# sevagh/Zen

Measured on AMD Instinct MI355X. Metric: hops/sec (1024-hop HPR, 44.1 kHz mono), higher is better.
Workload: dtype f32

## Files before the change

zen_amd/__init__.py:

```python
from .lib import (
    FREQUENCY, OUTPUT_HARMONIC, OUTPUT_PERCUSSIVE, OUTPUT_RESIDUAL, TIME_ANTICAUSAL, TIME_CAUSAL,
    BoxFilterGPU, DeviceBuffer, Event, FFTC2CWrapperGPU, HPR, HPRIOffline, HPRRealtime, IOGPU, MedianFilterGPU, PinnedHost,
    ZenHipError, ZgException, blockrun_set, blockrun_stats, debug_poke, device_name, init, load, memcheck, run_plan, set_option, synchronize,
)
from .addon_build import beat as beat_build, cqt as cqt_build, live as live_build, multi as multi_build, pcm as pcm_build, pitch as pitch_build, ragged as ragged_build, repet as repet_build, repsim as repsim_build
```

zen_amd/addon_build.py:

```python
import glob
import os
import subprocess
import sys
from concurrent.futures import ThreadPoolExecutor

HERE = os.path.dirname(os.path.abspath(__file__))
ROOT = os.path.dirname(HERE)
BASE = os.path.join(HERE, "libzen_hip.so")
HIPCC = os.environ.get("HIPCC", "/opt/rocm/bin/hipcc")
FLAGS = ["--offload-arch=gfx950", "-O3", "-std=c++17", "-fPIC", "-ffp-contract=off", "-fno-fast-math", "-Wall",
         "-I", os.path.join(ROOT, "include")]


class Addon:

    def __init__(self, name, sources, extra_deps=(), build_demo=None, title=None, file_flags=None):
        self.name, self.SOURCES, self.build_demo, self.title = name, list(sources), build_demo, title or name
        self.SRC = os.path.join(HERE, name)
        self.OUT = os.path.join(HERE, "libzen_hip_%s.so" % name)
        self.OBJDIR = os.path.join(HERE, "build_" + name)
        self.FLAGS = FLAGS
        self.FILE_FLAGS = dict(file_flags or {})
        self.extra_deps = [os.path.join(HERE, *d.split("/")) for d in extra_deps]

    def deps(self):
        hdrs = [os.path.join(self.SRC, f) for f in os.listdir(self.SRC) if f.endswith(".h")]
        hdrs += glob.glob(os.path.join(HERE, "addon", "*.h")) + self.extra_deps
        hdrs.append(os.path.join(ROOT, "include", "zen_hip.h"))
        hdrs.append(os.path.abspath(__file__))
        return hdrs

    def objects(self):
        return [os.path.join(self.OBJDIR, s.replace(".hip", ".o")) for s in self.SOURCES]

    def _compile(self, src):
        obj = os.path.join(self.OBJDIR, src.replace(".hip", ".o"))
        srcp = os.path.join(self.SRC, src)
        newest = max(os.path.getmtime(p) for p in [srcp] + self.deps())
        if os.path.exists(obj) and os.path.getmtime(obj) >= newest:
            return obj, False
        subprocess.check_call([HIPCC] + self.FLAGS + self.FILE_FLAGS.get(src, []) + ["-c", srcp, "-o", obj])
        return obj, True

    def build(self, force=False, verbose=False):
        if not os.path.exists(BASE):
            raise RuntimeError("%s not built: zen_amd/build.py first (the %s library links against it)" % (BASE, self.title))
        os.makedirs(self.OBJDIR, exist_ok=True)
        if force:
            for f in os.listdir(self.OBJDIR):
                os.remove(os.path.join(self.OBJDIR, f))
        with ThreadPoolExecutor(max_workers=len(self.SOURCES)) as ex:
            res = list(ex.map(self._compile, self.SOURCES))
        if any(r[1] for r in res) or not os.path.exists(self.OUT) or os.path.getmtime(self.OUT) < os.path.getmtime(BASE):
            subprocess.check_call([HIPCC, "--offload-arch=gfx950", "-shared", "-fPIC", "-o", self.OUT] + [r[0] for r in res]
                                  + ["-L", HERE, "-lzen_hip", "-Wl,-rpath,$ORIGIN"])
            if verbose:
                print("built", self.OUT)
        if self.build_demo:
            self.build_demo(verbose)
        return self.OUT


def _build_demo(name, source, exe, verbose):
    src, out = os.path.join(HERE, name), os.path.join(HERE, "libzen_hip_%s.so" % name)
    srcs = [os.path.join(src, source), os.path.join(src, "zen_hip_%s.h" % name), os.path.join(HERE, "cli", "wav.h"), out]
    if os.path.exists(exe) and os.path.getmtime(exe) >= max(os.path.getmtime(p) for p in srcs):
        return exe
    os.makedirs(os.path.dirname(exe), exist_ok=True)
    subprocess.check_call([os.environ.get("CXX", "g++"), "-std=c++17", "-O2", "-Wall", "-ffp-contract=off", "-I", os.path.join(ROOT, "include"),
                           "-I", src, "-I", os.path.join(HERE, "cli"), srcs[0], "-o", exe, "-L", HERE, "-lzen_hip_" + name, "-lzen_hip",
                           "-Wl,-rpath,$ORIGIN/.."])
    if verbose:
        print("built", exe)
    return exe


DEMO = os.path.join(HERE, "bin", "pitch-track")
BEAT_DEMO = os.path.join(HERE, "bin", "beat-track")
STEMS_DEMO = os.path.join(HERE, "bin", "zen-stems")
REPET_DEMO = os.path.join(HERE, "bin", "zen-repet")
CQT_DEMO = os.path.join(HERE, "bin", "zen-cqt")
REPSIM_DEMO = os.path.join(HERE, "bin", "zen-repsim")


def build_demo(verbose=False):
    return _build_demo("pitch", "pitch_track.cpp", DEMO, verbose)


def build_beat_demo(verbose=False):
    return _build_demo("beat", "beat_track.cpp", BEAT_DEMO, verbose)


def build_stems_demo(verbose=False):
    return _build_demo("multi", "multi_stems.cpp", STEMS_DEMO, verbose)


def build_repet_demo(verbose=False):
    return _build_demo("repet", "repet_main.cpp", REPET_DEMO, verbose)


def build_cqt_demo(verbose=False):
    return _build_demo("cqt", "cqt_main.cpp", CQT_DEMO, verbose)


def build_repsim_demo(verbose=False):
    return _build_demo("repsim", "repsim_main.cpp", REPSIM_DEMO, verbose)


pcm = Addon("pcm", ["pcm_kernels.hip", "pcm_pipe.hip"], extra_deps=["csrc/host_pipe.h"], title="PCM")
ragged = Addon("ragged", ["ragged_kernels.hip", "ragged.hip"])
live = Addon("live", ["live_kernels.hip", "live.hip"])
pitch = Addon("pitch", ["pitch_kernels.hip", "pitch.hip"], build_demo=build_demo)
ADDONS = {a.name: a for a in (pcm, ragged, live, pitch)}
blockrun = Addon("blockrun", ["blockrun_kernel.hip", "blockrun.hip"],
                 extra_deps=["csrc/hpr_engine.h", "csrc/rt_fused.h", "csrc/common.h", "csrc/bounds.h", "csrc/memguard.h", "csrc/masks.h",
                             "csrc/fft_dev.h", "csrc/median47_core.h", "csrc/median_net.h"],
                 file_flags={"blockrun_kernel.hip": ["-mllvm", "-amdgpu-sched-strategy=max-ilp", "-mllvm", "-amdgpu-use-amdgpu-trackers=1",
                                                     "-DZEN_FFT_LDS_BARRIER", "-DZEN_FFT_FOLD_ADDR", "-Wno-unused-function"]})
ENGINE_ADDONS = {blockrun.name: blockrun}
beat = Addon("beat", ["beat_kernels.hip", "beat.hip"], build_demo=build_beat_demo)
multi = Addon("multi", ["multi_kernels.hip", "multi.hip"], extra_deps=["pcm/pcm_convert.h"], build_demo=build_stems_demo)
repet = Addon("repet", ["repet_kernels.hip", "repet.hip"], build_demo=build_repet_demo)
cqt = Addon("cqt", ["cqt_kernels.hip", "cqt.hip"], build_demo=build_cqt_demo)
repsim = Addon("repsim", ["repsim_kernels.hip", "repsim.hip"], build_demo=build_repsim_demo)
LATER_ADDONS = {beat.name: beat, multi.name: multi, repet.name: repet, cqt.name: cqt, repsim.name: repsim}
ALL_ADDONS = {**ADDONS, **ENGINE_ADDONS, **LATER_ADDONS}


if __name__ == "__main__":
    names = [a for a in sys.argv[1:] if not a.startswith("--")] or list(ALL_ADDONS)
    for n in names:
        ALL_ADDONS[n].build(force="--force" in sys.argv, verbose=True)
```

zen_amd/blockrun/blockrun.hip:

```cpp
#include "../csrc/hpr_engine.h"
#include "../csrc/masks.h"
#include "blockrun_kernel.h"
#include "zen_hip_blockrun.h"

#include <atomic>
#include <cstring>

using namespace zen_hip_impl;

namespace {

std::atomic<int> g_run_len{0}, g_min_items{4096}, g_off{0};
std::atomic<unsigned long long> g_routed{0}, g_forwarded{0};

struct ProfScope {
	zen_hip_hpr* e;
	int k;
	hipEvent_t e0 = nullptr, e1 = nullptr;
	ProfScope(zen_hip_hpr* e_, int k_)
	    : e(e_)
	    , k(k_)
	{
		if (!e->prof)
			return;
		if (!e->prof_pool.empty()) {
			e0 = e->prof_pool.back().first;
			e1 = e->prof_pool.back().second;
			e->prof_pool.pop_back();
		}
		else if (hipEventCreate(&e0) != hipSuccess || hipEventCreate(&e1) != hipSuccess) {
			e0 = e1 = nullptr;
			return;
		}
		(void)hipEventRecord(e0, e->stream);
	}
	~ProfScope()
	{
		if (!e0)
			return;
		(void)hipEventRecord(e1, e->stream);
		e->prof_pending.push_back({k, e0, e1});
		e->prof_launches[k] += 1;
	}
};

int device_slots(int* slots)
{
	static std::atomic<int> cached[64];
	int dev = 0;
	ZH_HIP(hipGetDevice(&dev));
	int v = (dev >= 0 && dev < 64) ? cached[dev].load() : 0;
	if (v == 0) {
		int cus = 0;
		ZH_HIP(hipDeviceGetAttribute(&cus, hipDeviceAttributeMultiprocessorCount, dev));
		v = 3 * (cus > 0 ? cus : 1);
		if (dev >= 0 && dev < 64)
			cached[dev].store(v);
	}
	*slots = v;
	return ZEN_HIP_OK;
}

bool takes(const zen_hip_hpr* h, const float* in, size_t n_hops, size_t in_stride, const float* harm, const float* perc,
           const float* resid, size_t out_stride)
{
	if (g_off.load() || !h || !in || !perc || harm || resid || n_hops == 0)
		return false;
	if (h->causality != ZEN_HIP_TIME_CAUSAL || h->log2n != 12 || h->mf != zen_blockrun::TAPS || h->hop != (size_t)zen_blockrun::HOP
	    || h->nfft != (size_t)zen_blockrun::NFFT || h->nwin != 2 * h->hop)
		return false;
	if (!h->out_p || h->out_h || h->out_r || h->soft || h->use_sse)
		return false;
	if ((h->drain[0] | h->drain[1] | h->drain[2]) || h->rows_stale || h->run_mode || h->res_idle_ms != 0 || h->res_active || h->dbg_stamps)
		return false;
	if (!h->d_Y[0] || !h->d_blk_need || !h->d_carry[0] || !h->d_mag || n_hops > h->max_hops)
		return false;
	if (h->n_streams * n_hops < (size_t)g_min_items.load() || h->n_streams * n_hops > 0x3fffffffu)
		return false;
	int inc = 0;
	if (hard_mask_threshold(h->beta, &inc) == 0.0)
		return false;
	const size_t S = h->n_streams;
	const char *in0 = (const char*)in, *in1 = (const char*)(in + (S - 1) * in_stride + n_hops * h->hop);
	const char *o0 = (const char*)perc, *o1 = (const char*)(perc + (S - 1) * out_stride + n_hops * h->hop);
	return !(o0 < in1 && in0 < o1);
}

}

extern "C" int zen_hip_blockrun_process(zen_hip_hpr_t h, const float* in_dev, size_t n_hops, size_t in_stride, float* harm, float* perc,
                                        float* resid, size_t out_stride)
{
	if (!takes(h, in_dev, n_hops, in_stride, harm, perc, resid, out_stride)) {
		g_forwarded.fetch_add(1);
		return zen_hip_hpr_process(h, in_dev, n_hops, in_stride, harm, perc, resid, out_stride);
	}
	g_routed.fetch_add(1);
	int slots = 0;
	ZH_TRY(device_slots(&slots));
	zen_blockrun::RunArgs a;
	memset(&a, 0, sizeof(a));
	a.in = in_dev;
	a.in_stride = (long long)in_stride;
	a.tail_prev = h->d_tail[h->tail_sel];
	a.tail_next = h->d_tail[h->tail_sel ^ 1];
	a.window = h->d_window;
	a.tw = h->d_tw;
	a.mag = h->d_mag;
	a.keep_mag_rows = (int)h->W - 1;
	a.ring_rows = h->ring_rows;
	a.row0 = h->abs_frame;
	a.n_frames = (int)n_hops;
	a.n_streams = (int)h->n_streams;
	a.prev_frames = (int)h->last_frames;
	a.carry = h->d_carry[0];
	a.Y = h->d_Y[0];
	a.y_stream_stride = (long long)(h->max_hops * h->nwin);
	a.out = perc;
	a.out_stride = (long long)out_stride;
	a.need = h->d_blk_need;
	a.cola = h->cola;
	int inc = 0;
	a.thr = hard_mask_threshold(h->beta, &inc);
	a.part = zen_blockrun_partition(a.n_streams, a.n_frames, slots, g_run_len.load());
	for (int o = 0; o < 3; ++o) {
		h->ready_valid[o] = false;
		h->direct_done[o] = false;
	}
	{
		ProfScope ps(h, zen_hip_hpr::K_FUSED);
		ZH_TRY(zen_blockrun::launch_run(a, h->stream));
	}
	{
		ProfScope ps(h, zen_hip_hpr::K_FINALIZE);
		ZH_TRY(zen_blockrun::launch_fixup(a, h->stream));
	}
	h->tail_sel ^= 1;
	h->abs_frame += (long long)n_hops;
	h->last_frames = n_hops;
	return ZEN_HIP_OK;
}

extern "C" int zen_hip_blockrun_set(const char* key, int value)
{
	if (!key || value < 0)
		ZH_FAIL(ZEN_HIP_E_BAD_ARG, "blockrun_set: null key or negative value");
	if (!strcmp(key, "run_len"))
		g_run_len.store(value);
	else if (!strcmp(key, "min_items"))
		g_min_items.store(value);
	else if (!strcmp(key, "off"))
		g_off.store(value);
	else
		ZH_FAIL(ZEN_HIP_E_BAD_ARG, "blockrun_set: unknown key '%s' (run_len, min_items, off)", key);
	return ZEN_HIP_OK;
}

extern "C" int zen_hip_blockrun_stats(unsigned long long* routed, unsigned long long* forwarded)
{
	if (routed)
		*routed = g_routed.load();
	if (forwarded)
		*forwarded = g_forwarded.load();
	return ZEN_HIP_OK;
}
```

zen_amd/blockrun/blockrun_kernel.h:

```cpp
#pragma once
#include <hip/hip_runtime.h>

#include "blockrun_partition.h"

namespace zen_blockrun {

constexpr int HOP = 1024, NFFT = 4096, TAPS = 47;

struct RunArgs {
	const float* in;
	long long in_stride;
	const float* tail_prev;
	float* tail_next;
	const float* window;
	const float2* tw;
	float* mag;
	int keep_mag_rows;
	long long ring_rows, row0;
	int n_frames, n_streams, prev_frames;
	float* carry;
	float* Y;
	long long y_stream_stride;
	float* out;
	long long out_stride;
	unsigned* need;
	float cola;
	double thr;
	zen_blockrun_part part;
};

constexpr size_t LDS_BYTES_MAX = 53 * 1024;
size_t run_kernel_lds_bytes();
int launch_run(const RunArgs& a, hipStream_t stream);
int launch_fixup(const RunArgs& a, hipStream_t stream);

}
```

zen_amd/blockrun/blockrun_kernel.hip:

```cpp
#include "../csrc/common.h"
#include "../csrc/fft_dev.h"
#include "../csrc/masks.h"
#include "../csrc/median47_core.h"
#include "../csrc/median_net.h"
#include "blockrun_kernel.h"

#pragma clang fp contract(off)

namespace zen_blockrun {
namespace {

using zen_hip_impl::hard_mask_exact;
using PL = zfft::Plan<12>;
constexpr int N = PL::N, TF = PL::TF;
static_assert(N == NFFT && TF == 256 && HOP == 4 * TF, "four samples of a hop per thread");

constexpr int MID = TAPS / 2, MID_AL = 24, IMG_END = 255 * 16 + 64;
__device__ __forceinline__ int img_addr(int g) { return (g >> 4) * zm47::RSTR + (g & 15); }
constexpr int PC_WORD = 5184, PC_TAIL = 2052, EDGE_WORD = PC_WORD + PC_TAIL + 512 + 4;
static_assert((EDGE_WORD + 256) * 4 <= PL::LDS_FLOAT2 * 8, "lean layout must fit in the frame image");
constexpr int KEEP_WORD = PL::LDS_FLOAT2 * 2, CARRY_WORD = KEEP_WORD + HOP, WIN_WORD = CARRY_WORD + HOP;
constexpr size_t LDS_BYTES = (size_t)(WIN_WORD + 2 * HOP) * 4;
static_assert(LDS_BYTES <= LDS_BYTES_MAX, "three workgroups per CU");

__device__ __forceinline__ void lds_barrier()
{
	asm volatile("s_waitcnt lgkmcnt(0)\n\ts_barrier" ::: "memory");
}

struct TwGlobal32 {
	static constexpr bool PLAIN = true;
	static constexpr bool PACKED = true;
	const float2* __restrict__ p;
	__device__ __forceinline__ float2 get(int, int, int, int idx) const
	{
		return *reinterpret_cast<const float2*>(reinterpret_cast<const char*>(p) + (unsigned)(idx << 3));
	}
};

struct Spec {
	float2 S[16];
};

struct FwdInPre {
	float x[8], w[8];
	__device__ __forceinline__ float2 operator()(int, int slot) const { return make_float2(x[slot] * w[slot], 0.0f); }
};

struct FwdOut {
	Spec* r;
	int* img;
	__device__ __forceinline__ void operator()(int idx, float2 X, bool lower, int slot) const
	{
		r->S[slot] = X;
		if (lower || idx == (N >> 1)) {
			const float m = zfft::cabs_exact(X.x, X.y);
			const int key = __float_as_int(m);
			constexpr int CH = (TF / 16) * zm47::RSTR;
			const int tfl = idx - slot * TF;
			const int a0 = img_addr(tfl + MID_AL), a1 = img_addr(N - tfl + MID_AL);
			img[a0 + slot * CH] = key;
			img[(idx == 0 || idx == (N >> 1)) ? a0 + slot * CH : a1 - slot * CH] = key;
		}
	}
};

struct InvIn {
	const Spec* r;
	const int* img;
	const float* pc;
	double thr;
	__device__ __forceinline__ float2 operator()(int idx, int slot) const
	{
		const int lo = slot * TF, hi = lo + TF - 1;
		int pi;
		if (hi <= N / 2)
			pi = idx;
		else if (lo > N / 2 && hi < N - MID)
			pi = N - idx;
		else
			pi = (idx > N / 2 && idx < N - MID) ? N - idx : (idx > N / 2 ? idx - (N - 512) + PC_TAIL : idx);
		const int g0 = idx + 24 - slot * TF;
		const float mag = __int_as_float(img[(g0 >> 4) * 20 + (g0 & 15) + slot * (TF / 16) * 20]);
		const float2 z = r->S[slot];
		const float m = hard_mask_exact(pc[pi], mag + FLT_EPSILON, thr);
		return make_float2(z.x * m, z.y * m);
	}
};

struct InvOut {
	float* Y;
	float* out;
	float* carry;
	float cola;
	__device__ __forceinline__ void operator()(int idx, float2 x, bool, int slot) const
	{
		const float y = x.x * cola;
		ZH_CHK(Y + idx, 1);
		Y[idx] = y;
		if (slot < 4) {
			ZH_CHK(out + idx, 1);
			out[idx] = carry[(slot & 3) * TF] + y;
		}
		else {
			carry[(slot & 3) * TF] = y;
		}
	}
};

__global__ __launch_bounds__(256, 3) void blockrun_kernel(RunArgs a)
{
	extern __shared__ float2 lds[];
	int* img = reinterpret_cast<int*>(lds);
	float* Prow = reinterpret_cast<float*>(img + PC_WORD);
	const int tf = (int)threadIdx.x;
	float* keep = reinterpret_cast<float*>(img + KEEP_WORD) + tf;
	float* carry = reinterpret_cast<float*>(img + CARRY_WORD) + tf;
	float* win = reinterpret_cast<float*>(img + WIN_WORD) + tf;

	int s, f0, len;
	zen_blockrun_run(&a.part, (int)blockIdx.x, &s, &f0, &len);
	if (s >= a.n_streams || f0 + len > a.n_frames)
		return;
	const float* cur = a.in + (long long)s * a.in_stride + (long long)f0 * HOP;
	float* Yrow = a.Y + (long long)s * a.y_stream_stride + (long long)f0 * (2 * HOP);
	float* orow = a.out + (long long)s * a.out_stride + (long long)f0 * HOP;

	if (a.prev_frames > 0) {
		const int fc = a.prev_frames - 1 < a.n_frames - 1 ? a.prev_frames - 1 : a.n_frames - 1;
		if (fc >= f0 && fc < f0 + len) {
			const float* y = a.Y + (long long)s * a.y_stream_stride + (long long)(a.prev_frames - 1) * (2 * HOP) + HOP;
			float v[4];
#pragma unroll
			for (int i = 0; i < 4; ++i) {
				ZH_CHK(y + tf + i * TF, 1);
				v[i] = y[tf + i * TF];
			}
#pragma unroll
			for (int i = 0; i < 4; ++i) {
				ZH_CHK(a.carry + ((long long)s * HOP + tf + i * TF), 1);
				a.carry[(long long)s * HOP + tf + i * TF] = v[i];
			}
		}
	}
	float nx[4];
	{
		const float* pv = f0 > 0 ? cur - HOP : a.tail_prev + (long long)s * HOP;
		float p[4], w[8];
#pragma unroll
		for (int m = 0; m < 4; ++m) {
			ZH_CHK(pv + m * TF + tf, 1);
			ZH_CHK(cur + m * TF + tf, 1);
			p[m] = pv[m * TF + tf];
			nx[m] = cur[m * TF + tf];
		}
#pragma unroll
		for (int m = 0; m < 8; ++m) {
			ZH_CHK(a.window + m * TF + tf, 1);
			w[m] = a.window[m * TF + tf];
		}
#pragma unroll
		for (int m = 0; m < 4; ++m) {
			keep[m * TF] = p[m];
			carry[m * TF] = 0.0f;
		}
#pragma unroll
		for (int m = 0; m < 8; ++m)
			win[m * TF] = w[m];
	}
	if (tf == 0) {
		ZH_CHK(a.need + ((long long)s * a.n_frames + f0), 1);
		a.need[(long long)s * a.n_frames + f0] = 1u;
	}

	const int tf_run = tf;
	for (int k = 0; k < len; ++k) {
		const int f = f0 + k;
		int tf = tf_run, tw_off = 0;
		asm volatile("" : "+v"(tf));
		tf &= TF - 1;
		asm volatile("" : "+s"(tw_off));
		const float2* tw = a.tw + tw_off;
		float* keep = reinterpret_cast<float*>(img + KEEP_WORD) + tf;
		float* carry = reinterpret_cast<float*>(img + CARRY_WORD) + tf;
		float* win = reinterpret_cast<float*>(img + WIN_WORD) + tf;
		Spec r;
		{
			FwdInPre pre;
#pragma unroll
			for (int m = 0; m < 4; ++m) {
				pre.x[m] = keep[m * TF];
				pre.x[4 + m] = nx[m];
			}
#pragma unroll
			for (int m = 0; m < 8; ++m)
				pre.w[m] = win[m * TF];
#pragma unroll
			for (int m = 0; m < 4; ++m)
				keep[m * TF] = nx[m];
			if (f == a.n_frames - 1) {
				float* tail = a.tail_next + (long long)s * HOP;
#pragma unroll
				for (int m = 0; m < 4; ++m) {
					ZH_CHK(tail + m * TF + tf, 1);
					tail[m * TF + tf] = nx[m];
				}
			}
			FwdOut out;
			out.r = &r;
			out.img = img;
			zfft::PassRunner<12, 0, false, true, false, FwdInPre, FwdOut, false, TwGlobal32>::run(tf, lds, TwGlobal32{tw}, pre, out, true);
		}
		lds_barrier();
		if (f >= a.n_frames - a.keep_mag_rows) {
			float* mag = a.mag + (((a.row0 + f) % a.ring_rows) + (long long)s * a.ring_rows) * N;
			for (int g = tf; g < N; g += TF) {
				ZH_CHK(mag + g, 1);
				mag[g] = __int_as_float(img[img_addr(g + MID_AL)]);
			}
		}
		{
			const int v0 = img[img_addr(MID_AL)], v1 = img[img_addr(N - 1 + MID_AL)];
			for (int g = tf; g < MID_AL; g += TF)
				img[img_addr(g)] = v0;
			for (int g = N + MID_AL + tf; g < IMG_END; g += TF)
				img[img_addr(g)] = v1;
		}
		lds_barrier();
		{
			int(*edge)[64] = reinterpret_cast<int(*)[64]>(img + EDGE_WORD);
			const int lane = tf & 63, wave = __builtin_amdgcn_readfirstlane(tf >> 6);
			const int blk = wave < 2 ? tf : (lane < 32 ? 128 + lane : 192 + lane);
			zm47::Pieces pc;
			if (wave < 3)
				zm47::m47_sort_and_publish(img, edge, blk, lane, wave, tf == 0, blk == 255, pc);
			lds_barrier();
			if (wave < 3) {
				int o[16];
				zm47::m47_select(img, edge, blk, wave, pc, o);
				const int at = blk >= 224 ? PC_TAIL + (blk - 224) * 16 : blk * 16;
				if (blk <= 127 || blk >= 224) {
#pragma unroll
					for (int v = 0; v < 4; ++v)
						*reinterpret_cast<int4*>(&Prow[at + 4 * v]) = make_int4(o[4 * v], o[4 * v + 1], o[4 * v + 2], o[4 * v + 3]);
				}
				else if (blk == 128) {
					*reinterpret_cast<int4*>(&Prow[at]) = make_int4(o[0], o[1], o[2], o[3]);
				}
			}
		}
		lds_barrier();
		cur += HOP;
		if (k + 1 < len) {
#pragma unroll
			for (int m = 0; m < 4; ++m) {
				ZH_CHK(cur + m * TF + tf, 1);
				nx[m] = cur[m * TF + tf];
			}
		}
		{
			asm volatile("" : "+v"(tf));
			asm volatile("" : "+s"(tw_off));
			tf &= TF - 1;
			tw = a.tw + tw_off;
			carry = reinterpret_cast<float*>(img + CARRY_WORD) + tf;
			InvIn in;
			in.r = &r;
			in.img = img;
			in.pc = Prow;
			in.thr = a.thr;
			InvOut out;
			out.Y = Yrow;
			out.out = orow;
			out.carry = carry;
			out.cola = a.cola;
			zfft::PassRunner<12, 0, true, false, true, InvIn, InvOut, true, TwGlobal32>::run(tf, lds, TwGlobal32{tw}, in, out, true);
		}
		Yrow += 2 * HOP;
		orow += HOP;
	}
}

__global__ __launch_bounds__(256) void blockrun_fixup_kernel(RunArgs a)
{
	const long long total = (long long)a.n_streams * a.n_frames;
	const long long item = (long long)blockIdx.x * 4 + (threadIdx.x >> 6);
	const int lane = threadIdx.x & 63;
	if (item >= total)
		return;
	ZH_CHK(a.need + item, 1);
	if (!a.need[item])
		return;
	const int s = (int)(item / a.n_frames), f = (int)(item - (long long)s * a.n_frames);
	const float* Y = a.Y + (long long)s * a.y_stream_stride + (long long)f * (2 * HOP);
	const float* prev = f == 0 ? a.carry + (long long)s * HOP : Y - HOP;
	float* o = a.out + (long long)s * a.out_stride + (long long)f * HOP;
	if (((reinterpret_cast<uintptr_t>(o) | reinterpret_cast<uintptr_t>(prev) | reinterpret_cast<uintptr_t>(Y)) & 15) == 0) {
		float4 p[HOP / 256], y[HOP / 256];
#pragma unroll
		for (int i = 0; i < HOP / 256; ++i) {
			const int k = i * 256 + lane * 4;
			ZH_CHK(prev + k, 4);
			ZH_CHK(Y + k, 4);
			p[i] = *reinterpret_cast<const float4*>(prev + k);
			y[i] = *reinterpret_cast<const float4*>(Y + k);
		}
#pragma unroll
		for (int i = 0; i < HOP / 256; ++i) {
			const int k = i * 256 + lane * 4;
			ZH_CHK(o + k, 4);
			*reinterpret_cast<float4*>(o + k) = make_float4(p[i].x + y[i].x, p[i].y + y[i].y, p[i].z + y[i].z, p[i].w + y[i].w);
		}
	}
	else {
		for (int k = lane; k < HOP; k += 64) {
			ZH_CHK(o + k, 1);
			ZH_CHK(prev + k, 1);
			ZH_CHK(Y + k, 1);
			o[k] = prev[k] + Y[k];
		}
	}
	if (lane == 0)
		a.need[item] = 0u;
}

}

size_t run_kernel_lds_bytes() { return LDS_BYTES; }

int launch_run(const RunArgs& a, hipStream_t stream)
{
	const long long runs = (long long)a.n_streams * a.part.runs_per_stream;
	hipLaunchKernelGGL(blockrun_kernel, dim3((unsigned)runs), dim3(TF), LDS_BYTES, stream, a);
	ZH_HIP(hipGetLastError());
	return ZEN_HIP_OK;
}

int launch_fixup(const RunArgs& a, hipStream_t stream)
{
	const long long total = (long long)a.n_streams * a.n_frames;
	hipLaunchKernelGGL(blockrun_fixup_kernel, dim3((unsigned)((total + 3) / 4)), dim3(256), 0, stream, a);
	ZH_HIP(hipGetLastError());
	return ZEN_HIP_OK;
}

}
```

zen_amd/blockrun/zen_hip_blockrun.h:

```cpp
#ifndef ZEN_HIP_BLOCKRUN_H
#define ZEN_HIP_BLOCKRUN_H

#include <stddef.h>

#include "zen_hip.h"

#ifdef __cplusplus
extern "C" {
#endif

int zen_hip_blockrun_process(zen_hip_hpr_t h, const float* in_dev, size_t n_hops, size_t in_stride, float* harm, float* perc,
                             float* resid, size_t out_stride);

int zen_hip_blockrun_set(const char* key, int value);

int zen_hip_blockrun_stats(unsigned long long* routed, unsigned long long* forwarded);

#ifdef __cplusplus
}
#endif

#endif
```

zen_amd/lib.py:

```python
import ctypes as C
import os

import numpy as np

_HERE = os.path.dirname(os.path.abspath(__file__))
_SO = os.environ.get("ZEN_HIP_SO") or os.path.join(_HERE, "libzen_hip.so")

TIME_CAUSAL, TIME_ANTICAUSAL, FREQUENCY = 0, 1, 2
OUTPUT_HARMONIC, OUTPUT_PERCUSSIVE, OUTPUT_RESIDUAL = 1, 2, 4
E_FILTER_TOO_BIG, E_BAD_ARG, E_HOPS_NOT_DIVISIBLE, E_HIP, E_UNSUPPORTED = 1, 2, 3, 4, 5


class ZenHipError(RuntimeError):
    def __init__(self, code, msg):
        self.code = code
        super().__init__("zen_hip error %d: %s" % (code, msg))


class ZgException(ZenHipError):
    """Raised where the reference throws zen::ZgException (libzen/libzen/zen.h:8-12)."""


class _Params(C.Structure):
    _fields_ = [("hop", C.c_size_t), ("nwin", C.c_size_t), ("nfft", C.c_size_t),
# ... 66 lines not shown
    ("zen_hip_hpr_process_next_hop", _i, [_vp, _vp]),
    ("zen_hip_hpr_copy_output", _i, [_vp, _u, _vp]),
    ("zen_hip_hpr_copy_output_async", _i, [_vp, _u, _vp]),
    ("zen_hip_hpr_process", _i, [_vp, _vp, _sz, _sz, _vp, _vp, _vp, _sz]),
    ("zen_hip_hpr_process_host", _i, [_vp, _vp, _sz, _vp, _vp, _vp]),
    ("zen_hip_hpr_debug_stamps", _i, [_vp, C.POINTER(C.POINTER(C.c_ulonglong))]),
    ("zen_hip_hpr_profile", _i, [_vp, _i]),
    ("zen_hip_hpr_profile_get", _i, [_vp, C.POINTER(C.c_double), C.POINTER(C.c_ulonglong),
                                     C.POINTER(C.c_ulonglong)]),
    ("zen_hip_hpr_profile_get_all", _i, [_vp, C.POINTER(C.c_double), C.POINTER(C.c_ulonglong)]),
    ("zen_hip_hpri_create", _i, [_f, _sz, _sz, _f, _f, _i, _sz, _pvp]),
    ("zen_hip_hpri_destroy", _i, [_vp]),
    ("zen_hip_hpri_set_stream", _i, [_vp, _vp]),
    ("zen_hip_hpri_use_sse_filter", _i, [_vp]),
    ("zen_hip_hpri_use_soft_mask", _i, [_vp]),
    ("zen_hip_hpri_process", _i, [_vp, _vp, _sz, _vp, _vp, _vp]),
    ("zen_hip_hpri_process_sink", _i, [_vp, _vp, _sz, _i, _i, _vp, _vp]),
    ("zen_hip_hpri_host_stats_get", _i, [_vp, C.POINTER(_HostStats)]),
    ("zen_hip_hpri_process_device", _i, [_vp, _vp, _sz, _sz, _vp, _vp, _vp, _sz]),
    ("zen_hip_hpri_range_halo", _i, [_vp, _sz, _sz, _sz, C.POINTER(_sz), C.POINTER(_sz)]),
    ("zen_hip_hpri_process_range", _i, [_vp, _vp, _sz, _sz, _sz, _vp, _vp]),
    ("zen_hip_hpri_hop_counts", _i, [_vp, _sz, C.POINTER(_sz), C.POINTER(_sz)]),
    ("zen_hip_run_plan", _i, [_sz, _sz, _sz, C.POINTER(C.c_int), C.c_int, C.POINTER(C.c_int), C.POINTER(C.c_double)]),
    ("zen_hip_hpri_profile", _i, [_vp, _i]),
    ("zen_hip_hpri_profile_get_all", _i, [_vp, _i, C.POINTER(C.c_double), C.POINTER(C.c_ulonglong)]),
]

_lib = None


def load():
    global _lib
    if _lib is None:
        if not os.path.exists(_SO):
            raise ImportError("%s not built: run `python zen_amd/build.py` (needs hipcc)" % _SO)
        L = C.CDLL(_SO)
        for name, res, args in SYMBOLS:
            f = getattr(L, name)
            f.restype = res
            f.argtypes = args
        _lib = L
    return _lib


def _ck(rc):
    if rc:
        msg = load().zen_hip_last_error().decode()
        if rc in (E_FILTER_TOO_BIG, E_HOPS_NOT_DIVISIBLE):
            raise ZgException(rc, msg)
        raise ZenHipError(rc, msg)


def init(device=0):
    _ck(load().zen_hip_init(device))
    for item in filter(None, os.environ.get("ZEN_HIP_OPTIONS", "").split(",")):
        name, _, val = item.partition("=")
        set_option(name.strip(), int(val or 1))


class Event:

    def __init__(self):
        e = C.c_void_p()
        _ck(load().zen_hip_event_create(C.byref(e)))
        self._e = e.value

    def record(self, stream=None):
        _ck(load().zen_hip_event_record(self._e, stream))

    def elapsed_ms(self, stop):
        ms = C.c_float()
        _ck(load().zen_hip_event_elapsed_ms(self._e, stop._e, C.byref(ms)))
        return ms.value

    def __del__(self):
        if getattr(self, "_e", None):
            load().zen_hip_event_destroy(self._e)
            self._e = None


def synchronize(stream=None):
    _ck(load().zen_hip_synchronize(stream))


def run_plan(frames, streams, nfft, group_outputs=(2, 1)):
    g = (C.c_int * len(group_outputs))(*group_outputs)
    run, busy = C.c_int(), C.c_double()
    _ck(load().zen_hip_run_plan(frames, streams, nfft, g, len(group_outputs), C.byref(run), C.byref(busy)))
    return run.value, busy.value


def memcheck():
    r = _MemcheckReport()
    _ck(load().zen_hip_memcheck(C.byref(r)))
    d = {k: getattr(r, k) for k, _ in _MemcheckReport._fields_}
    d["first_message"] = d["first_message"].decode(errors="replace")
    d["first_violation"] = d["first_violation"].decode(errors="replace")
    return d


def debug_poke(dev_ptr, byte_offset, value):
    _ck(load().zen_hip_debug_poke(dev_ptr, int(byte_offset), int(value) & 0xFFFFFFFF))


_BASE_ONLY_OPTIONS = ("no_block_fused", "no_rt_fused", "no_direct_out", "mask_divide", "rt_fused_diag")
_options = {}


def set_option(name, value):
    _ck(load().zen_hip_set_option(name.encode(), int(value)))
    _options[name] = int(value)


BLOCKRUN_SYMBOLS = [
    ("zen_hip_blockrun_process", _i, [_vp, _vp, _sz, _sz, _vp, _vp, _vp, _sz]),
    ("zen_hip_blockrun_set", _i, [C.c_char_p, _i]),
    ("zen_hip_blockrun_stats", _i, [C.POINTER(C.c_ulonglong), C.POINTER(C.c_ulonglong)]),
]
_blockrun = None


def load_blockrun():
    global _blockrun
    if _blockrun is None:
        import subprocess
        from . import _addon
        try:
            _blockrun = _addon.load("blockrun", BLOCKRUN_SYMBOLS)
        except (ImportError, OSError, RuntimeError, subprocess.CalledProcessError):
            _blockrun = False
        else:
            for item in filter(None, os.environ.get("ZEN_HIP_BLOCKRUN", "").split(",")):
                name, _, val = item.partition("=")
                blockrun_set(name.strip(), int(val or 1))
    return _blockrun


def blockrun_set(key, value):
    L = load_blockrun()
    if not L:
        raise ImportError("libzen_hip_blockrun.so is not built and cannot be built here")
    _ck(L.zen_hip_blockrun_set(key.encode(), int(value)))


def blockrun_stats():
    L = load_blockrun()
    if not L:
        raise ImportError("libzen_hip_blockrun.so is not built and cannot be built here")
    a, b = C.c_ulonglong(), C.c_ulonglong()
    _ck(L.zen_hip_blockrun_stats(C.byref(a), C.byref(b)))
    return a.value, b.value


def device_name():
    buf = C.create_string_buffer(256)
    _ck(load().zen_hip_device_name(buf, 256))
    return buf.value.decode()


class DeviceBuffer:

    def __init__(self, n, dtype=np.float32):
        self.n, self.dtype = int(n), np.dtype(dtype)
        p = C.c_void_p()
        _ck(load().zen_hip_malloc(C.byref(p), self.n * self.dtype.itemsize))
        self.ptr = p.value

    @classmethod
    def from_host(cls, a):
        a = np.ascontiguousarray(a)
        b = cls(a.size, a.dtype)
        b.upload(a)
        return b

    def upload(self, a):
        a = np.ascontiguousarray(a, dtype=self.dtype)
        assert a.size <= self.n
        _ck(load().zen_hip_memcpy_h2d(self.ptr, a.ctypes.data, a.size * self.dtype.itemsize))

    def download(self, n=None):
        n = self.n if n is None else n
        out = np.empty(n, self.dtype)
        _ck(load().zen_hip_memcpy_d2h(out.ctypes.data, self.ptr, n * self.dtype.itemsize))
        return out

    def zero(self):
        _ck(load().zen_hip_memset(self.ptr, 0, self.n * self.dtype.itemsize, None))

    def offset(self, n_elems):
        return self.ptr + n_elems * self.dtype.itemsize

    def free(self):
        if getattr(self, "ptr", None):
            load().zen_hip_free(self.ptr)
            self.ptr = None

    def __del__(self):
        self.free()


class IOGPU:

    def __init__(self, size):
        self.size = size
        hi, di, ho, do = C.c_void_p(), C.c_void_p(), C.c_void_p(), C.c_void_p()
        _ck(load().zen_hip_host_alloc_mapped(size * 4, 1, C.byref(hi), C.byref(di)))
        _ck(load().zen_hip_host_alloc_mapped(size * 4, 0, C.byref(ho), C.byref(do)))
        self._hi, self._ho = hi.value, ho.value
        self.device_in, self.device_out = di.value, do.value
        self.host_in = np.ctypeslib.as_array(C.cast(hi, C.POINTER(C.c_float)), shape=(size,))
        self.host_out = np.ctypeslib.as_array(C.cast(ho, C.POINTER(C.c_float)), shape=(size,))

    def __del__(self):
        if getattr(self, "_hi", None):
            load().zen_hip_host_free(self._hi)
            load().zen_hip_host_free(self._ho)
            self._hi = None


class PinnedHost:

    def __init__(self, n):
        h, d = C.c_void_p(), C.c_void_p()
        _ck(load().zen_hip_host_alloc_mapped(n * 4, 0, C.byref(h), C.byref(d)))
        self._h = h.value
        self.array = np.ctypeslib.as_array(C.cast(h, C.POINTER(C.c_float)), shape=(n,))

    def free(self):
        if getattr(self, "_h", None):
            self.array = None
            load().zen_hip_host_free(self._h)
            self._h = None

    def __del__(self):
        self.free()


class FFTC2CWrapperGPU:

    def __init__(self, nfft):
        self.nfft = nfft
        h = C.c_void_p()
        _ck(load().zen_hip_fft_create(nfft, C.byref(h)))
        self._h = h.value
        self.fft_vec = DeviceBuffer(nfft, np.complex64)
        self.fft_vec.zero()

    def forward(self):
        _ck(load().zen_hip_fft_exec(self._h, self.fft_vec.ptr, 0, None))

    def backward(self):
        _ck(load().zen_hip_fft_exec(self._h, self.fft_vec.ptr, 1, None))

    def exec_batched(self, dev_ptr, batch, inverse=False):
        _ck(load().zen_hip_fft_exec_batched(self._h, dev_ptr, batch, int(inverse), None))

    def __del__(self):
        if getattr(self, "_h", None):
            load().zen_hip_fft_destroy(self._h)
            self._h = None


class _Filter:
    _kind = None

    def __init__(self, time, frequency, filter_len, direction, copy_bord=False):
        self.time, self.frequency, self.filter_len, self.direction = time, frequency, filter_len, direction
        h = C.c_void_p()
        L = load()
        if self._kind == "mfilt":
            _ck(L.zen_hip_mfilt_create(time, frequency, filter_len, direction, int(copy_bord), C.byref(h)))
        else:
            _ck(L.zen_hip_box_create(time, frequency, filter_len, direction, C.byref(h)))
        self._h = h.value

    def assume_nonneg(self, on=True):
        _ck(load().zen_hip_mfilt_assume_nonneg(self._h, int(bool(on))))

    def filter(self, src, dst):
        s = src.ptr if isinstance(src, DeviceBuffer) else src
        d = dst.ptr if isinstance(dst, DeviceBuffer) else dst
        L = load()
        _ck((L.zen_hip_mfilt_run if self._kind == "mfilt" else L.zen_hip_box_run)(self._h, s, d, None))

    def filter_host(self, a):
        a = np.ascontiguousarray(a, dtype=np.float32)
        assert a.shape == (self.time, self.frequency)
        src, dst = DeviceBuffer.from_host(a), DeviceBuffer(a.size)
        dst.zero()
        self.filter(src, dst)
        synchronize()
        return dst.download().reshape(a.shape)

    def __del__(self):
        if getattr(self, "_h", None):
            L = load()
            (L.zen_hip_mfilt_destroy if self._kind == "mfilt" else L.zen_hip_box_destroy)(self._h)
            self._h = None


class MedianFilterGPU(_Filter):
    _kind = "mfilt"


class BoxFilterGPU(_Filter):
    _kind = "box"
# ... 221 lines not shown
```

Measured before the change: 57.51 million.

## Skip redundant mirror stores, fold border fill into FFT output, add pow2 mask path

The forward FFT output stores each magnitude once, plus a mirror copy only where the median windows actually read it. The border replication is written with vector stores inside the output functor, which removes a separate fill pass and one LDS barrier per frame. The inverse input reads mirrored magnitudes through the twin-column mapping. A templated kernel variant uses a cheaper float comparison for the hard mask when beta is a power of two. An optional stamps build adds cycle-counter instrumentation, which risks layout subtleties and adds code paths to maintain.

```diff
diff --git a/zen_amd/__init__.py b/zen_amd/__init__.py
--- a/zen_amd/__init__.py
+++ b/zen_amd/__init__.py
@@ -1,6 +1,6 @@
 from .lib import (
     FREQUENCY, OUTPUT_HARMONIC, OUTPUT_PERCUSSIVE, OUTPUT_RESIDUAL, TIME_ANTICAUSAL, TIME_CAUSAL,
     BoxFilterGPU, DeviceBuffer, Event, FFTC2CWrapperGPU, HPR, HPRIOffline, HPRRealtime, IOGPU, MedianFilterGPU, PinnedHost,
-    ZenHipError, ZgException, blockrun_set, blockrun_stats, debug_poke, device_name, init, load, memcheck, run_plan, set_option, synchronize,
+    ZenHipError, ZgException, blockrun_mask_stats, blockrun_set, blockrun_stats, debug_poke, device_name, init, load, memcheck, run_plan, set_option, synchronize,
 )
 from .addon_build import beat as beat_build, cqt as cqt_build, live as live_build, multi as multi_build, pcm as pcm_build, pitch as pitch_build, ragged as ragged_build, repet as repet_build, repsim as repsim_build
diff --git a/zen_amd/addon_build.py b/zen_amd/addon_build.py
--- a/zen_amd/addon_build.py
+++ b/zen_amd/addon_build.py
@@ -14,12 +14,13 @@
 
 class Addon:
 
-    def __init__(self, name, sources, extra_deps=(), build_demo=None, title=None, file_flags=None):
+    def __init__(self, name, sources, extra_deps=(), build_demo=None, title=None, file_flags=None, variant=None, variant_flags=()):
         self.name, self.SOURCES, self.build_demo, self.title = name, list(sources), build_demo, title or name
         self.SRC = os.path.join(HERE, name)
-        self.OUT = os.path.join(HERE, "libzen_hip_%s.so" % name)
-        self.OBJDIR = os.path.join(HERE, "build_" + name)
-        self.FLAGS = FLAGS
+        tag = name + ("_" + variant if variant else "")
+        self.OUT = os.path.join(HERE, "libzen_hip_%s.so" % tag)
+        self.OBJDIR = os.path.join(HERE, "build_" + tag)
+        self.FLAGS = FLAGS + list(variant_flags) if variant else FLAGS
         self.FILE_FLAGS = dict(file_flags or {})
         self.extra_deps = [os.path.join(HERE, *d.split("/")) for d in extra_deps]
 
@@ -112,12 +113,14 @@
 live = Addon("live", ["live_kernels.hip", "live.hip"])
 pitch = Addon("pitch", ["pitch_kernels.hip", "pitch.hip"], build_demo=build_demo)
 ADDONS = {a.name: a for a in (pcm, ragged, live, pitch)}
-blockrun = Addon("blockrun", ["blockrun_kernel.hip", "blockrun.hip"],
+_BLOCKRUN = dict(sources=["blockrun_kernel.hip", "blockrun.hip"],
                  extra_deps=["csrc/hpr_engine.h", "csrc/rt_fused.h", "csrc/common.h", "csrc/bounds.h", "csrc/memguard.h", "csrc/masks.h",
                              "csrc/fft_dev.h", "csrc/median47_core.h", "csrc/median_net.h"],
                  file_flags={"blockrun_kernel.hip": ["-mllvm", "-amdgpu-sched-strategy=max-ilp", "-mllvm", "-amdgpu-use-amdgpu-trackers=1",
                                                      "-DZEN_FFT_LDS_BARRIER", "-DZEN_FFT_FOLD_ADDR", "-Wno-unused-function"]})
+blockrun = Addon("blockrun", **_BLOCKRUN)
 ENGINE_ADDONS = {blockrun.name: blockrun}
+blockrun_stamps = Addon("blockrun", variant="stamps", variant_flags=["-DZEN_BLOCKRUN_STAMPS"], **_BLOCKRUN)
 beat = Addon("beat", ["beat_kernels.hip", "beat.hip"], build_demo=build_beat_demo)
 multi = Addon("multi", ["multi_kernels.hip", "multi.hip"], extra_deps=["pcm/pcm_convert.h"], build_demo=build_stems_demo)
 repet = Addon("repet", ["repet_kernels.hip", "repet.hip"], build_demo=build_repet_demo)
diff --git a/zen_amd/blockrun/blockrun.hip b/zen_amd/blockrun/blockrun.hip
--- a/zen_amd/blockrun/blockrun.hip
+++ b/zen_amd/blockrun/blockrun.hip
@@ -1,6 +1,7 @@
 #include "../csrc/hpr_engine.h"
 #include "../csrc/masks.h"
 #include "blockrun_kernel.h"
+#include "blockrun_mask.h"
 #include "zen_hip_blockrun.h"
 
 #include <atomic>
@@ -11,7 +12,11 @@
 namespace {
 
 std::atomic<int> g_run_len{0}, g_min_items{4096}, g_off{0};
-std::atomic<unsigned long long> g_routed{0}, g_forwarded{0};
+std::atomic<unsigned long long> g_routed{0}, g_forwarded{0}, g_pow2{0}, g_general{0};
+#ifdef ZEN_BLOCKRUN_STAMPS
+std::atomic<unsigned long long*> g_stamps{nullptr};
+std::atomic<int> g_stamp_groups{0}, g_stamp_frames{0};
+#endif
 
 struct ProfScope {
 	zen_hip_hpr* e;
@@ -122,7 +127,14 @@
 	a.cola = h->cola;
 	int inc = 0;
 	a.thr = hard_mask_threshold(h->beta, &inc);
+	a.beta_pow2 = zen_blockrun_beta_pow2(h->beta) ? h->beta : 0.0f;
+	(a.beta_pow2 != 0.0f ? g_pow2 : g_general).fetch_add(1);
 	a.part = zen_blockrun_partition(a.n_streams, a.n_frames, slots, g_run_len.load());
+#ifdef ZEN_BLOCKRUN_STAMPS
+	a.stamps = g_stamps.load();
+	a.stamp_groups = g_stamp_groups.load();
+	a.stamp_frames = g_stamp_frames.load();
+#endif
 	for (int o = 0; o < 3; ++o) {
 		h->ready_valid[o] = false;
 		h->direct_done[o] = false;
@@ -156,6 +168,28 @@
 	return ZEN_HIP_OK;
 }
 
+extern "C" int zen_blockrun_mask_stats(unsigned long long* pow2, unsigned long long* general)
+{
+	if (pow2)
+		*pow2 = g_pow2.load();
+	if (general)
+		*general = g_general.load();
+	return ZEN_HIP_OK;
+}
+
+#ifdef ZEN_BLOCKRUN_STAMPS
+extern "C" int zen_blockrun_set_stamps(unsigned long long* buf, int groups, int frames)
+{
+	if (buf && (groups <= 0 || frames <= 0))
+		ZH_FAIL(ZEN_HIP_E_BAD_ARG, "blockrun_set_stamps: a buffer of %d groups of %d frames", groups, frames);
+	g_stamps.store(nullptr);
+	g_stamp_groups.store(buf ? groups : 0);
+	g_stamp_frames.store(buf ? frames : 0);
+	g_stamps.store(buf);
+	return ZEN_HIP_OK;
+}
+#endif
+
 extern "C" int zen_hip_blockrun_stats(unsigned long long* routed, unsigned long long* forwarded)
 {
 	if (routed)
diff --git a/zen_amd/blockrun/blockrun_kernel.h b/zen_amd/blockrun/blockrun_kernel.h
--- a/zen_amd/blockrun/blockrun_kernel.h
+++ b/zen_amd/blockrun/blockrun_kernel.h
@@ -26,8 +26,17 @@
 	unsigned* need;
 	float cola;
 	double thr;
+	float beta_pow2;
 	zen_blockrun_part part;
+#ifdef ZEN_BLOCKRUN_STAMPS
+	unsigned long long* stamps;
+	int stamp_groups, stamp_frames;
+#endif
 };
+
+#ifdef ZEN_BLOCKRUN_STAMPS
+constexpr int STAMP_WORDS = 10, STAMP_EVERY = 64;
+#endif
 
 constexpr size_t LDS_BYTES_MAX = 53 * 1024;
 size_t run_kernel_lds_bytes();
diff --git a/zen_amd/blockrun/blockrun_kernel.hip b/zen_amd/blockrun/blockrun_kernel.hip
--- a/zen_amd/blockrun/blockrun_kernel.hip
+++ b/zen_amd/blockrun/blockrun_kernel.hip
@@ -4,6 +4,8 @@
 #include "../csrc/median47_core.h"
 #include "../csrc/median_net.h"
 #include "blockrun_kernel.h"
+#include "blockrun_layout.h"
+#include "blockrun_mask.h"
 
 #pragma clang fp contract(off)
 
@@ -16,7 +18,13 @@
 static_assert(N == NFFT && TF == 256 && HOP == 4 * TF, "four samples of a hop per thread");
 
 constexpr int MID = TAPS / 2, MID_AL = 24, IMG_END = 255 * 16 + 64;
-__device__ __forceinline__ int img_addr(int g) { return (g >> 4) * zm47::RSTR + (g & 15); }
+__device__ __forceinline__ int img_addr(int g) { return zen_blockrun_img_addr(g); }
+__device__ __forceinline__ int twin_col(int k) { return zen_blockrun_twin_col(k); }
+static_assert(ZBL_N == N && ZBL_TF == TF && ZBL_MID == MID && ZBL_MID_AL == MID_AL && ZBL_RSTR == zm47::RSTR && ZBL_IMG_END == IMG_END, "one layout");
+static_assert(ZBL_UP_LO_END == 2087 && ZBL_MIRROR7_TF == 217 && ZBL_UP_HI_BEGIN == 4040 && ZBL_MIRROR0_TF == 56, "the kept mirror stores");
+static_assert(16 * ZBL_LAST_LOW_BLK + 3 + MID <= ZBL_UP_LO_END && 16 * ZBL_LAST_LOW_BLK == N / 2, "block 128's four used medians see columns up to N/2 + 3 + 23");
+static_assert(16 * ZBL_FIRST_HIGH_BLK <= N - MID && N - MID < 16 * (ZBL_FIRST_HIGH_BLK + 1) && ZBL_UP_HI_BEGIN <= N - MID - MID, "bin N - 23 is in block 254");
+static_assert(ZBL_MIRROR7_TF > 0 && ZBL_MIRROR7_TF < TF && ZBL_MIRROR0_TF < TF && (N + MID_AL) % 16 == 8 && IMG_END % 16 == 0, "mirror conditions and 16-byte border stores");
 constexpr int PC_WORD = 5184, PC_TAIL = 2052, EDGE_WORD = PC_WORD + PC_TAIL + 512 + 4;
 static_assert((EDGE_WORD + 256) * 4 <= PL::LDS_FLOAT2 * 8, "lean layout must fit in the frame image");
 constexpr int KEEP_WORD = PL::LDS_FLOAT2 * 2, CARRY_WORD = KEEP_WORD + HOP, WIN_WORD = CARRY_WORD + HOP;
@@ -38,6 +46,25 @@
 	}
 };
 
+#ifdef ZEN_BLOCKRUN_STAMPS
+struct Stamp {
+	unsigned long long* p;
+	__device__ __forceinline__ void operator()(int i) const
+	{
+		if (p)
+			p[i] = __builtin_readcyclecounter();
+	}
+	__device__ __forceinline__ void wall(int i) const
+	{
+		if (p)
+			p[i] = wall_clock64();
+	}
+};
+#define ZB_STAMP(i) stamp(i)
+#else
+#define ZB_STAMP(i) ((void)0)
+#endif
+
 struct Spec {
 	float2 S[16];
 };
@@ -53,23 +80,40 @@
 	__device__ __forceinline__ void operator()(int idx, float2 X, bool lower, int slot) const
 	{
 		r->S[slot] = X;
-		if (lower || idx == (N >> 1)) {
+		constexpr int CH = (TF / 16) * zm47::RSTR;
+		const int tfl = idx - slot * TF;
+		if (lower) {
 			const float m = zfft::cabs_exact(X.x, X.y);
 			const int key = __float_as_int(m);
-			constexpr int CH = (TF / 16) * zm47::RSTR;
-			const int tfl = idx - slot * TF;
-			const int a0 = img_addr(tfl + MID_AL), a1 = img_addr(N - tfl + MID_AL);
-			img[a0 + slot * CH] = key;
-			img[(idx == 0 || idx == (N >> 1)) ? a0 + slot * CH : a1 - slot * CH] = key;
-		}
-	}
-};
-
+			img[img_addr(tfl + MID_AL) + slot * CH] = key;
+			if (zen_blockrun_keeps_mirror(slot, tfl))
+				img[img_addr(N - tfl + MID_AL) - slot * CH] = key;
+			if (slot == 0 && tfl < 2) {
+				const int4 q = make_int4(key, key, key, key);
+				const int g0 = tfl == 0 ? 0 : N + MID_AL;
+#pragma unroll
+				for (int w = 0; w < MID_AL; w += 4)
+					*reinterpret_cast<int4*>(img + img_addr(g0 + w)) = q;
+			}
+		}
+		else if (slot == 8 && tfl == 0) {
+			img[img_addr(MID_AL) + slot * CH] = __float_as_int(zfft::cabs_exact(X.x, X.y));
+		}
+	}
+};
+
+__device__ __forceinline__ float hard_mask_pow2(float x, float d, float beta) { return zen_blockrun_hard_mask_pow2(x, d, beta); }
+
+template <bool POW2>
 struct InvIn {
 	const Spec* r;
 	const int* img;
 	const float* pc;
 	double thr;
+	float beta;
+#ifdef ZEN_BLOCKRUN_STAMPS
+	Stamp stamp;
+#endif
 	__device__ __forceinline__ float2 operator()(int idx, int slot) const
 	{
 		const int lo = slot * TF, hi = lo + TF - 1;
@@ -80,10 +124,13 @@
 			pi = N - idx;
 		else
 			pi = (idx > N / 2 && idx < N - MID) ? N - idx : (idx > N / 2 ? idx - (N - 512) + PC_TAIL : idx);
-		const int g0 = idx + 24 - slot * TF;
-		const float mag = __int_as_float(img[(g0 >> 4) * 20 + (g0 & 15) + slot * (TF / 16) * 20]);
+		constexpr int CH = (TF / 16) * zm47::RSTR;
+		const int tfl = idx - slot * TF;
+		const float mag = __int_as_float(img[slot < 8 ? img_addr(tfl + MID_AL) + slot * CH : img_addr(MID_AL - tfl) + (16 - slot) * CH]);
 		const float2 z = r->S[slot];
-		const float m = hard_mask_exact(pc[pi], mag + FLT_EPSILON, thr);
+		const float m = POW2 ? hard_mask_pow2(pc[pi], mag + FLT_EPSILON, beta) : hard_mask_exact(pc[pi], mag + FLT_EPSILON, thr);
+		if (slot == 15)
+			ZB_STAMP(5);
 		return make_float2(z.x * m, z.y * m);
 	}
 };
@@ -108,6 +155,7 @@
 	}
 };
 
+template <bool POW2>
 __global__ __launch_bounds__(256, 3) void blockrun_kernel(RunArgs a)
 {
 	extern __shared__ float2 lds[];
@@ -176,6 +224,18 @@
 	const int tf_run = tf;
 	for (int k = 0; k < len; ++k) {
 		const int f = f0 + k;
+#ifdef ZEN_BLOCKRUN_STAMPS
+		Stamp stamp;
+		{
+			const int grp = (int)blockIdx.x / STAMP_EVERY;
+			const bool on = a.stamps && (int)blockIdx.x % STAMP_EVERY == 0 && grp < a.stamp_groups && k < a.stamp_frames && threadIdx.x == 0;
+			stamp.p = on ? a.stamps + ((long long)grp * a.stamp_frames + k) * STAMP_WORDS : nullptr;
+			if (on)
+				stamp.p[9] = (unsigned long long)len;
+		}
+		stamp.wall(7);
+		ZB_STAMP(0);
+#endif
 		int tf = tf_run, tw_off = 0;
 		asm volatile("" : "+v"(tf));
 		tf &= TF - 1;
@@ -211,22 +271,16 @@
 			out.img = img;
 			zfft::PassRunner<12, 0, false, true, false, FwdInPre, FwdOut, false, TwGlobal32>::run(tf, lds, TwGlobal32{tw}, pre, out, true);
 		}
+		ZB_STAMP(1);
 		lds_barrier();
 		if (f >= a.n_frames - a.keep_mag_rows) {
 			float* mag = a.mag + (((a.row0 + f) % a.ring_rows) + (long long)s * a.ring_rows) * N;
 			for (int g = tf; g < N; g += TF) {
 				ZH_CHK(mag + g, 1);
-				mag[g] = __int_as_float(img[img_addr(g + MID_AL)]);
-			}
-		}
-		{
-			const int v0 = img[img_addr(MID_AL)], v1 = img[img_addr(N - 1 + MID_AL)];
-			for (int g = tf; g < MID_AL; g += TF)
-				img[img_addr(g)] = v0;
-			for (int g = N + MID_AL + tf; g < IMG_END; g += TF)
-				img[img_addr(g)] = v1;
-		}
-		lds_barrier();
+				mag[g] = __int_as_float(img[img_addr(twin_col(g) + MID_AL)]);
+			}
+		}
+		ZB_STAMP(2);
 		{
 			int(*edge)[64] = reinterpret_cast<int(*)[64]>(img + EDGE_WORD);
 			const int lane = tf & 63, wave = __builtin_amdgcn_readfirstlane(tf >> 6);
@@ -234,6 +288,7 @@
 			zm47::Pieces pc;
 			if (wave < 3)
 				zm47::m47_sort_and_publish(img, edge, blk, lane, wave, tf == 0, blk == 255, pc);
+			ZB_STAMP(3);
 			lds_barrier();
 			if (wave < 3) {
 				int o[16];
@@ -249,6 +304,7 @@
 				}
 			}
 		}
+		ZB_STAMP(4);
 		lds_barrier();
 		cur += HOP;
 		if (k + 1 < len) {
@@ -264,20 +320,28 @@
 			tf &= TF - 1;
 			tw = a.tw + tw_off;
 			carry = reinterpret_cast<float*>(img + CARRY_WORD) + tf;
-			InvIn in;
+			InvIn<POW2> in;
 			in.r = &r;
 			in.img = img;
 			in.pc = Prow;
 			in.thr = a.thr;
+			in.beta = a.beta_pow2;
+#ifdef ZEN_BLOCKRUN_STAMPS
+			in.stamp = stamp;
+#endif
 			InvOut out;
 			out.Y = Yrow;
 			out.out = orow;
 			out.carry = carry;
 			out.cola = a.cola;
-			zfft::PassRunner<12, 0, true, false, true, InvIn, InvOut, true, TwGlobal32>::run(tf, lds, TwGlobal32{tw}, in, out, true);
+			zfft::PassRunner<12, 0, true, false, true, InvIn<POW2>, InvOut, true, TwGlobal32>::run(tf, lds, TwGlobal32{tw}, in, out, true);
 		}
 		Yrow += 2 * HOP;
 		orow += HOP;
+#ifdef ZEN_BLOCKRUN_STAMPS
+		ZB_STAMP(6);
+		stamp.wall(8);
+#endif
 	}
 }
 
@@ -331,7 +395,10 @@
 int launch_run(const RunArgs& a, hipStream_t stream)
 {
 	const long long runs = (long long)a.n_streams * a.part.runs_per_stream;
-	hipLaunchKernelGGL(blockrun_kernel, dim3((unsigned)runs), dim3(TF), LDS_BYTES, stream, a);
+	if (a.beta_pow2 != 0.0f)
+		hipLaunchKernelGGL(blockrun_kernel<true>, dim3((unsigned)runs), dim3(TF), LDS_BYTES, stream, a);
+	else
+		hipLaunchKernelGGL(blockrun_kernel<false>, dim3((unsigned)runs), dim3(TF), LDS_BYTES, stream, a);
 	ZH_HIP(hipGetLastError());
 	return ZEN_HIP_OK;
 }
diff --git a/zen_amd/blockrun/blockrun_layout.h b/zen_amd/blockrun/blockrun_layout.h
--- /dev/null
+++ b/zen_amd/blockrun/blockrun_layout.h
@@ -0,0 +1,34 @@
+#ifndef ZEN_HIP_BLOCKRUN_LAYOUT_H
+#define ZEN_HIP_BLOCKRUN_LAYOUT_H
+
+#include "blockrun_partition.h"
+
+enum {
+	ZBL_N = 4096, ZBL_TF = 256, ZBL_MID = 23, ZBL_MID_AL = 24, ZBL_RSTR = 20,
+	ZBL_IMG_END = 255 * 16 + 64,
+	ZBL_LAST_LOW_BLK = 128,
+	ZBL_FIRST_HIGH_BLK = 254,
+	ZBL_UP_LO_END = 16 * (ZBL_LAST_LOW_BLK + 3) - 9,
+	ZBL_UP_HI_BEGIN = 16 * ZBL_FIRST_HIGH_BLK - 24,
+	ZBL_MIRROR7_TF = ZBL_N - ZBL_UP_LO_END - 7 * ZBL_TF,
+	ZBL_MIRROR0_TF = ZBL_N - ZBL_UP_HI_BEGIN
+};
+
+ZEN_BLOCKRUN_FN int zen_blockrun_img_addr(int g) { return (g >> 4) * ZBL_RSTR + (g & 15); }
+
+ZEN_BLOCKRUN_FN int zen_blockrun_twin_col(int k) { return k > ZBL_N / 2 ? ZBL_N - k : k; }
+
+ZEN_BLOCKRUN_FN int zen_blockrun_keeps_mirror(int slot, int tf)
+{
+	return (slot == 7 && tf >= ZBL_MIRROR7_TF) || (slot == 0 && tf >= 1 && tf <= ZBL_MIRROR0_TF);
+}
+
+ZEN_BLOCKRUN_FN int zen_blockrun_invin_word(int slot, int tf)
+{
+	const int ch = (ZBL_TF / 16) * ZBL_RSTR;
+	if (slot < 8)
+		return zen_blockrun_img_addr(tf + ZBL_MID_AL) + slot * ch;
+	return zen_blockrun_img_addr(ZBL_MID_AL - tf) + (16 - slot) * ch;
+}
+
+#endif
diff --git a/zen_amd/blockrun/blockrun_mask.h b/zen_amd/blockrun/blockrun_mask.h
--- /dev/null
+++ b/zen_amd/blockrun/blockrun_mask.h
@@ -0,0 +1,24 @@
+#ifndef ZEN_HIP_BLOCKRUN_MASK_H
+#define ZEN_HIP_BLOCKRUN_MASK_H
+
+#include <math.h>
+#include <string.h>
+
+#include "blockrun_partition.h"
+
+static inline int zen_blockrun_beta_pow2(float beta)
+{
+	unsigned u;
+	unsigned expo;
+	memcpy(&u, &beta, sizeof(u));
+	expo = (u >> 23) & 0xffu;
+	return (u >> 31) == 0 && expo >= 127u && expo != 0xffu && (u & 0x7fffffu) == 0;
+}
+
+ZEN_BLOCKRUN_FN float zen_blockrun_hard_mask_pow2(float x, float d, float beta)
+{
+	const float t = fmaxf(beta * d, 0x1p-149f) + (d - d);
+	return x >= t ? 1.0f : 0.0f;
+}
+
+#endif
diff --git a/zen_amd/blockrun/zen_hip_blockrun.h b/zen_amd/blockrun/zen_hip_blockrun.h
--- a/zen_amd/blockrun/zen_hip_blockrun.h
+++ b/zen_amd/blockrun/zen_hip_blockrun.h
@@ -16,6 +16,8 @@
 
 int zen_hip_blockrun_stats(unsigned long long* routed, unsigned long long* forwarded);
 
+int zen_blockrun_mask_stats(unsigned long long* pow2, unsigned long long* general);
+
 #ifdef __cplusplus
 }
 #endif
diff --git a/zen_amd/lib.py b/zen_amd/lib.py
--- a/zen_amd/lib.py
+++ b/zen_amd/lib.py
@@ -242,6 +242,17 @@
     return a.value, b.value
 
 
+def blockrun_mask_stats():
+    L = load_blockrun()
+    if not L:
+        raise ImportError("libzen_hip_blockrun.so is not built and cannot be built here")
+    f = L.zen_blockrun_mask_stats
+    f.restype, f.argtypes = _i, [C.POINTER(C.c_ulonglong), C.POINTER(C.c_ulonglong)]
+    a, b = C.c_ulonglong(), C.c_ulonglong()
+    _ck(f(C.byref(a), C.byref(b)))
+    return a.value, b.value
+
+
 def device_name():
     buf = C.create_string_buffer(256)
     _ck(load().zen_hip_device_name(buf, 256))
```

New measurement: 57.76 million (median of 6 runs). Within noise of the previous version (+0.4%).
